# AsherBond/0-kno-blobstreamx

Hardware: AMD Instinct MI355X
Metric: Goldilocks NTT GB/s @ 2^20–2^24 (higher is better)
Workload: dtype u64; 1 GPU; forward NTT, n=2^20, batch=128 per GPU, in place, natural order (BASELINE configs[1] wires shape); log_n=20, batch_per_gpu=128, plan=strip(R=2^10,C=2^4,E=32)+finalT(R=2^10,C=2^3,E=32), plan_is_the_bit_exact_tested_plan=True

## Files before the change

### 0-kno-blobstreamx_amd/csrc/gl_field.cuh

```cuda
#pragma once
#include <stdint.h>

#if defined(__HIPCC__)
#define GL_HD __host__ __device__ __forceinline__
#else
#define GL_HD inline __attribute__((always_inline))
#endif

typedef uint64_t u64;
typedef uint32_t u32;

#define GL_P 0xFFFFFFFF00000001ULL
#define GL_EPS 0xFFFFFFFFULL

template <int V> struct glp_ic { static constexpr int value = V; };
template <int I, int N, class F>
GL_HD void glp_static_for(F&& f) {
    if constexpr (I < N) {
        f(glp_ic<I>{});
        glp_static_for<I + 1, N>(f);
    }
}

#if defined(__HIP_DEVICE_COMPILE__) && !defined(GLP_EMU) && !defined(GLP_NO_ASM_FIELD)
#define GLP_ASM_FIELD 1
#else
#define GLP_ASM_FIELD 0
#endif

GL_HD u64 gl_make64(u32 lo, u32 hi) { return ((u64)hi << 32) | lo; }

GL_HD u64 gl_add_u32(u64 x, u32 y) {
#if GLP_ASM_FIELD
    u64 r, junk;
    asm("v_mad_u64_u32 %0, %1, %2, 1, %3" : "=v"(r), "=s"(junk) : "v"(y), "v"(x));
    return r;
#else
    return x + (u64)y;
#endif
}

GL_HD u64 gl_add(u64 a, u64 b) {
    const u64 s = a + b;
    const bool over = (s < a) | (s >= GL_P);
    return s + (over ? GL_EPS : 0ULL);
}

GL_HD u64 gl_sub(u64 a, u64 b) {
#if GLP_ASM_FIELD
    u32 dl, dh;
    u64 K;
    asm("v_sub_co_u32 %0, vcc, %3, %5\n\t"
        "v_subb_co_u32 %1, vcc, %4, %6, vcc\n\t"
        "v_addc_co_u32 %0, %2, 0, %0, vcc\n\t"
        "s_andn2_b64 vcc, vcc, %2\n\t"
        "v_subbrev_co_u32 %1, %2, 0, %1, vcc"
        : "=&v"(dl), "=&v"(dh), "=&s"(K)
        : "v"((u32)a), "v"((u32)(a >> 32)), "v"((u32)b), "v"((u32)(b >> 32))
        : "scc", "vcc");
    return gl_make64(dl, dh);
#else
    u64 d = a - b;
    return (a < b) ? d - GL_EPS : d;
#endif
}

template <bool CANON>
GL_HD u64 gl_mad_eps(u32 w, u64 t) {
#if GLP_ASM_FIELD
    u64 r;
    u32 m;
    if constexpr (CANON) {
        u64 G, J;
        asm("v_mad_u64_u32 %0, vcc, %4, -1, %5\n\t"
            "v_cmp_le_u64 %1, %6, %0\n\t"
            "s_or_b64 vcc, vcc, %1\n\t"
            "s_nop 0\n\t"
            "v_cndmask_b32 %2, 0, -1, vcc\n\t"
            "v_mad_u64_u32 %0, %3, %2, 1, %0"
            : "=&v"(r), "=&s"(G), "=&v"(m), "=&s"(J)
            : "v"(w), "v"(t), "s"(GL_P)
            : "scc", "vcc");
    } else {
        u64 J;
        asm("v_mad_u64_u32 %0, vcc, %3, -1, %4\n\t"
            "v_cndmask_b32 %1, 0, -1, vcc\n\t"
            "v_mad_u64_u32 %0, %2, %1, 1, %0"
            : "=&v"(r), "=&v"(m), "=&s"(J)
            : "v"(w), "v"(t)
            : "vcc");
    }
    return r;
#else
    const u64 t1 = ((u64)w << 32) - w;
    u64 r;
    const bool c = __builtin_add_overflow(t, t1, &r);
    if (CANON) return r + ((c | (r >= GL_P)) ? GL_EPS : 0ULL);
    return r + (c ? GL_EPS : 0ULL);
#endif
}
GL_HD u64 gl_neg(u64 a) { return a ? GL_P - a : 0; }
GL_HD u64 gl_canon(u64 a) { return a >= GL_P ? a - GL_P : a; }

GL_HD u64 gl_fold_carry(u64 r, bool carry) { return r + ((carry | (r >= GL_P)) ? GL_EPS : 0ULL); }

template <bool CANON>
GL_HD u64 gl_reduce128_t(u64 hi, u64 lo) {
    const u32 h0 = (u32)hi, h1 = (u32)(hi >> 32);
#if GLP_ASM_FIELD
    u32 tl, th;
    u64 K;
    asm("v_sub_co_u32 %0, vcc, %3, %5\n\t"
        "v_subbrev_co_u32 %1, vcc, 0, %4, vcc\n\t"
        "v_addc_co_u32 %0, %2, 0, %0, vcc\n\t"
        "s_andn2_b64 vcc, vcc, %2\n\t"
        "v_subbrev_co_u32 %1, %2, 0, %1, vcc"
        : "=&v"(tl), "=&v"(th), "=&s"(K)
        : "v"((u32)lo), "v"((u32)(lo >> 32)), "v"(h1)
        : "scc", "vcc");
    return gl_mad_eps<CANON>(h0, gl_make64(tl, th));
#else
    u64 t0;
    const bool bor = __builtin_sub_overflow(lo, (u64)h1, &t0);
    t0 = bor ? t0 + GL_P : t0;
    return gl_mad_eps<CANON>(h0, t0);
#endif
}
GL_HD u64 gl_reduce128(u64 hi, u64 lo) { return gl_reduce128_t<true>(hi, lo); }

template <bool CANON>
GL_HD u64 gl_mul_t(u64 a, u64 b) {
#if !defined(__HIP_DEVICE_COMPILE__) && !defined(GLP_EMU) && defined(__SIZEOF_INT128__)
    const unsigned __int128 p = (unsigned __int128)a * b;
    return gl_reduce128_t<CANON>((u64)(p >> 64), (u64)p);
#else
    const u32 a0 = (u32)a, a1 = (u32)(a >> 32), b0 = (u32)b, b1 = (u32)(b >> 32);
    const u64 p0 = (u64)a0 * b0;
    const u64 p1 = (u64)a0 * b1 + (p0 >> 32);
    const u64 p2 = (u64)a1 * b0 + (u32)p1;
    const u64 p3 = gl_add_u32((u64)a1 * b1 + (p1 >> 32), (u32)(p2 >> 32));
    return gl_reduce128_t<CANON>(p3, (p2 << 32) | (u32)p0);
#endif
}
GL_HD u64 gl_mul(u64 a, u64 b) { return gl_mul_t<true>(a, b); }
GL_HD u64 gl_sqr(u64 a) { return gl_mul(a, a); }

GL_HD u64 gl_fold_small(u64 al, u64 ah) {
#if GLP_ASM_FIELD
    u32 lh, m;
    u64 C1, J, v;
    asm("v_add_co_u32 %0, %1, %2, %3" : "=v"(lh), "=s"(C1) : "v"((u32)(al >> 32)), "v"((u32)ah));
    asm("v_mad_u64_u32 %0, vcc, %3, -1, %4\n\t"
        "s_or_b64 vcc, vcc, %5\n\t"
        "s_nop 0\n\t"
        "v_cndmask_b32 %1, 0, -1, vcc\n\t"
        "v_mad_u64_u32 %0, %2, %1, 1, %0"
        : "=&v"(v), "=&v"(m), "=&s"(J)
        : "v"((u32)(ah >> 32)), "v"(gl_make64((u32)al, lh)), "s"(C1)
        : "scc", "vcc");
    return v;
#else
    const u64 l = al + (ah << 32);
    const bool c1 = l < al;
    const u64 t = (ah >> 32) * GL_EPS;
    const u64 v = l + t;
    const bool c2 = v < l;
    return v + ((c1 | c2) ? GL_EPS : 0ULL);
#endif
}

GL_HD u64 gl_mul_nc(u64 a, u64 b) { return gl_mul_t<false>(a, b); }

template <int T>
GL_HD u64 gl_shl_small(u64 x) {
    static_assert(T > 0 && T < 32, "");
    return gl_mad_eps<true>((u32)(x >> (64 - T)), x << T);
}
template <int K>
GL_HD u64 gl_shr_small(u64 x) {
    static_assert(K > 0 && K <= 32, "");
    const u32 m = (K == 32) ? (0u - (u32)x) : ((0u - (u32)x) & ((1u << (K & 31)) - 1u));
    const u64 a = (x + m) >> (K & 63);
    const u32 mm = (K == 32) ? m : (m << ((32 - K) & 31));
    return a + (((u64)mm << 32) - mm);
}
GL_HD u64 gl_shl32(u64 x) { return gl_mad_eps<true>((u32)(x >> 32), x << 32); }

constexpr bool gl_pow2_neg(int S) {
    const int e = S % 96;
    const bool flip = (e > 32);
    return ((S / 96) & 1) != (flip ? 1 : 0);
}
template <int S>
GL_HD u64 gl_mul_pow2_mag(u64 x) {
    static_assert(S >= 0 && S < 192, "shift out of range");
    constexpr int e = S % 96;
    if constexpr (e == 0) return x;
    else if constexpr (e < 32) return gl_shl_small<e>(x);
    else if constexpr (e == 32) return gl_shl32(x);
    else if constexpr (e < 64) return gl_shr_small<32>(gl_shr_small<64 - e>(x));
    else return gl_shr_small<96 - e>(x);
}
template <int S>
GL_HD u64 gl_mul_pow2(u64 x) {
    const u64 v = gl_mul_pow2_mag<S>(x);
    if constexpr (gl_pow2_neg(S)) return gl_neg(v);
    else return v;
}

GL_HD u64 gl_pow(u64 a, u64 e) {
    u64 r = 1;
    while (e) {
        if (e & 1) r = gl_mul(r, a);
        a = gl_mul(a, a);
        e >>= 1;
    }
    return r;
}
GL_HD u64 gl_inv(u64 a) { return gl_pow(a, GL_P - 2); }
#ifndef GLP_TWO_ADIC_GENERATOR
#define GLP_TWO_ADIC_GENERATOR 1753635133440165772ULL
#endif
#ifndef GLP_W64_LOG2
#define GLP_W64_LOG2 39
#endif
static_assert(GLP_W64_LOG2 > 0 && GLP_W64_LOG2 < 192 && GLP_W64_LOG2 % 3 == 0 && GLP_W64_LOG2 % 2 == 1, "w_64 = 2^e needs e an odd multiple of 3");
GL_HD u64 gl_root_of_unity(unsigned k) { return gl_pow(GLP_TWO_ADIC_GENERATOR, 1ULL << (32 - k)); }

struct gl_ext2 { u64 a, b; };
GL_HD gl_ext2 gl_ext_add(gl_ext2 x, gl_ext2 y) { return {gl_add(x.a, y.a), gl_add(x.b, y.b)}; }
GL_HD gl_ext2 gl_ext_sub(gl_ext2 x, gl_ext2 y) { return {gl_sub(x.a, y.a), gl_sub(x.b, y.b)}; }
GL_HD gl_ext2 gl_ext_mul(gl_ext2 x, gl_ext2 y) {
    u64 bb = gl_mul(x.b, y.b);
    u64 w = gl_add(gl_add(gl_add(bb, bb), gl_add(bb, bb)), gl_add(gl_add(bb, bb), bb));
    return {gl_add(gl_mul(x.a, y.a), w), gl_add(gl_mul(x.a, y.b), gl_mul(x.b, y.a))};
}
GL_HD gl_ext2 gl_ext_scale(gl_ext2 x, u64 s) { return {gl_mul(x.a, s), gl_mul(x.b, s)}; }
```

### 0-kno-blobstreamx_amd/csrc/ntt_kernels.cuh

```cuda
#pragma once
#include "gl_field.cuh"
#include "ntt_plan.h"

constexpr int glp_bitrev_c(int v, int bits) {
    int r = 0;
    for (int i = 0; i < bits; i++) r |= ((v >> i) & 1) << (bits - 1 - i);
    return r;
}
constexpr int glp_tw_exp(int m, int i, bool inv) {
    int e = (GLP_W64_LOG2 * (64 / m) * i) % 192;
    return inv ? (192 - e) % 192 : e;
}

template <int Q, bool INV, int OFF, int NX>
GL_HD void glp_dft_inreg(u64 (&x)[NX]) {
    glp_static_for<0, Q>([&](auto s_) {
        constexpr int s = decltype(s_)::value;
        constexpr int half = 1 << (Q - 1 - s);
        constexpr int m = 2 * half;
        glp_static_for<0, (1 << Q) / 2>([&](auto t_) {
            constexpr int t = decltype(t_)::value;
            constexpr int blk = t / half, i = t % half;
            constexpr int i0 = OFF + blk * m + i, i1 = i0 + half;
            constexpr int e = glp_tw_exp(m, i, INV);
            u64 u = x[i0], v = x[i1];
            x[i0] = gl_add(u, v);
            if constexpr (gl_pow2_neg(e)) x[i1] = gl_mul_pow2_mag<e>(gl_sub(v, u));
            else x[i1] = gl_mul_pow2_mag<e>(gl_sub(u, v));
        });
    });
}


struct GlpNttPassArgs {
    const u64* src;
    u64* dst;
    u64 src_poly_stride;
    u64 dst_poly_stride;
    const u64* tw_tile;
    const u64* tw_lo;
    const u64* tw_hi;
    u64 scale;
    u32 log_n;
    u32 log_m;
    u32 log_c;
    u32 batch;
    u32 rev;
    u32 nprev;
    u32 log_rprev[3];
    u32 xcd_group_log;
    const u64* tw_full;
    u32 poly_minor;
    u32 coset_log;
    u32 src_coset;
    const u64* in_row;
    const u64* in_col;
};

static inline bool glp_ntt_args_plain(const GlpNttPassArgs& a) {
    return !a.coset_log && !a.src_coset && !a.in_row && !a.in_col && !a.tw_full && !a.poly_minor && !a.rev;
}

template <int LOG_R, int LOG_E>
struct GlpSteps {
    static constexpr int S = (LOG_R + LOG_E - 1) / LOG_E;
    static constexpr int q(int t) { return t == 0 ? LOG_R - LOG_E * (S - 1) : LOG_E; }
    static constexpr int log_sigma(int t) { return LOG_E * (S - 1 - t); }
    static constexpr int low_bits(int t) { return t == 0 ? 0 : q(0) + LOG_E * (t - 1); }
};

template <int LOG_R, int LOG_E>
GL_HD u32 glp_digit_reverse(u32 pos) {
    using ST = GlpSteps<LOG_R, LOG_E>;
    u32 k = 0;
    glp_static_for<0, ST::S>([&](auto t_) {
        constexpr int t = decltype(t_)::value;
        u32 digit = (pos >> ST::log_sigma(t)) & ((1u << ST::q(t)) - 1u);
        k |= digit << ST::low_bits(t);
    });
    return k;
}

GL_HD u32 glp_bitrev32(u32 v, u32 bits) {
    if (bits == 0) return 0;
#if defined(__HIP_DEVICE_COMPILE__)
    return __brev(v) >> (32 - bits);
#else
    u32 r = 0;
    for (u32 i = 0; i < bits; i++) r |= ((v >> i) & 1u) << (bits - 1 - i);
    return r;
#endif
}

#if defined(GLP_EMU)
#define GLP_DYN_LDS(name) u64* name = reinterpret_cast<u64*>(glp_emu_dyn_lds())
#else
#define GLP_DYN_LDS(name) extern __shared__ __attribute__((aligned(16))) u64 name[]
#endif

template <int LOG_E, int MODE> struct GlpSplit { static constexpr bool value = (LOG_E >= 5 && MODE != GLP_FINAL_ROWS); };

template <int LOG_E, int MODE, int CT_LOG_C = -1> struct GlpBounds {
    static constexpr int threads = LOG_E == 6 ? 512 : ((LOG_E == 5 && MODE == GLP_FINAL_T) ? 256 : 1024);
    static constexpr int waves = LOG_E == 6 ? 2 : (LOG_E == 5 ? (MODE == GLP_FINAL_T ? 3 : 4) : 1);
};
template <int LOG_R, int MODE, bool INV, int LOG_E = 4, bool PLAIN = false, int CT_LOG_C = -1>
__global__ void __launch_bounds__((GlpBounds<LOG_E, MODE, CT_LOG_C>::threads), (GlpBounds<LOG_E, MODE, CT_LOG_C>::waves)) glp_ntt_pass_kernel(GlpNttPassArgs a) {
    static_assert(!PLAIN || MODE != GLP_FINAL_ROWS, "FINAL_ROWS has no plain form");
    using ST = GlpSteps<LOG_R, LOG_E>;
    const u32 a_coset_log = PLAIN ? 0u : a.coset_log;
    const u32 a_src_coset = PLAIN ? 0u : a.src_coset;
    const u64* const a_in_row = PLAIN ? nullptr : a.in_row;
    const u64* const a_in_col = PLAIN ? nullptr : a.in_col;
    const u64* const a_tw_full = PLAIN ? nullptr : a.tw_full;
    const u32 a_poly_minor = PLAIN ? 0u : a.poly_minor;
    const u32 a_rev = PLAIN ? 0u : a.rev;
    constexpr u32 R = 1u << LOG_R;
    constexpr u32 E = 1u << LOG_E;
    constexpr bool SPLIT = GlpSplit<LOG_E, MODE>::value;
    GLP_DYN_LDS(lds);
    u32* const lds32 = reinterpret_cast<u32*>(lds);

    const u32 log_c = CT_LOG_C >= 0 ? (u32)CT_LOG_C : a.log_c;
    const u32 C = 1u << log_c;
    const u32 NT = (R << log_c) >> LOG_E;
    const u32 tid = threadIdx.x;
    const u32 ldA = C + 1;
    u64 tile = blockIdx.x;
    if constexpr (MODE == GLP_STRIP || MODE == GLP_FINAL_T) {
        const u32 g = a.xcd_group_log;
        if (g) {
            const u64 per = 8ull << g;
            const u64 base = tile & ~(per - 1);
            const u32 rem = (u32)(tile & (per - 1));
            tile = base + ((u64)(rem & 7u) << g) + (rem >> 3);
        }
    }

    auto poly_off = [&](u64 v, u64 stride, bool blocked) -> u64 {
        if (!a_coset_log) return v * stride;
        const u32 kc = (u32)v & ((1u << a_coset_log) - 1u);
        return (v >> a_coset_log) * stride + (blocked ? ((u64)glp_bitrev32(kc, a_coset_log) << a.log_n) : 0ull);
    };
    const u32 coset_mask = (1u << a_coset_log) - 1u;

    u64 sbase = 0, dbase = 0;
    u32 lo0 = 0, kcos = 0;
    u64 row_first = 0;
    const u32 log_rows = a.log_n - LOG_R;
    if constexpr (MODE == GLP_STRIP) {
        const u32 log_tpp = a.log_n - LOG_R - log_c;
        u64 poly;
        u32 t;
        if (a_poly_minor) {
            const u32 g = a.xcd_group_log;
            const u64 rest = tile >> g;
            poly = rest % a.batch;
            t = (u32)(((rest / a.batch) << g) | (tile & ((1ull << g) - 1)));
        } else {
            poly = tile >> log_tpp;
            t = (u32)(tile & ((1ull << log_tpp) - 1));
        }
        const u32 log_mc = a.log_m - log_c;
        const u32 hi = t >> log_mc;
        lo0 = (t & ((1u << log_mc) - 1u)) << log_c;
        const u64 off = ((u64)hi << (LOG_R + a.log_m)) + lo0;
        sbase = poly_off(poly, a.src_poly_stride, a_src_coset != 0) + off;
        dbase = poly_off(poly, a.dst_poly_stride, true) + off;
        kcos = (u32)poly & coset_mask;
    } else {
        row_first = tile << log_c;
    }
    const u64 total_rows = (u64)a.batch << log_rows;

    u64 x[E];

    auto unit_geom = [&](auto T_, u32 g, u32& col, u32& row0, u32& o_lo) {
        constexpr int T = decltype(T_)::value;
        constexpr int q = ST::q(T);
        constexpr int lsg = ST::log_sigma(T);
        const u32 u = g * NT + tid;
        u32 o;
        if (T == 0 && MODE != GLP_STRIP) {
            o = u & ((R >> q) - 1u);
            col = u >> (LOG_R - q);
        } else {
            col = u & (C - 1u);
            o = u >> log_c;
        }
        o_lo = o & ((1u << lsg) - 1u);
        row0 = ((o >> lsg) << (q + lsg)) | o_lo;
    };

    glp_static_for<0, ST::S>([&](auto t_) {
        constexpr int t = decltype(t_)::value;
        constexpr int q = ST::q(t);
        constexpr u32 r = 1u << q;
        constexpr int lsg = ST::log_sigma(t);
        constexpr u32 G = E / r;
        constexpr bool first = (t == 0), last = (t == ST::S - 1);

        u32 colv[G], row0v[G], olov[G];
        glp_static_for<0, (int)G>([&](auto g_) {
            constexpr int g = decltype(g_)::value;
            u32 col, row0, o_lo;
            unit_geom(t_, (u32)g, col, row0, o_lo);
            colv[g] = col; row0v[g] = row0; olov[g] = o_lo;
            if constexpr (first) {
                if constexpr (MODE == GLP_STRIP) {
                    const u64* const ps = a.src + (sbase + col + ((u64)row0 << a.log_m));
                    const u64 st = 1ull << (lsg + a.log_m);
                    glp_static_for<0, (int)r>([&](auto d_) {
                        constexpr int d = decltype(d_)::value;
                        x[g * r + d] = ps[(u64)d * st];
                    });
                    if (a_in_row) {
                        u64 sc[r];
                        glp_static_for<0, (int)r>([&](auto d_) {
                            constexpr int d = decltype(d_)::value;
                            sc[d] = a_in_row[(kcos << LOG_R) + row0 + ((u32)d << lsg)];
                        });
                        glp_static_for<0, (int)r>([&](auto d_) {
                            constexpr int d = decltype(d_)::value;
                            x[g * r + d] = gl_mul(x[g * r + d], sc[d]);
                        });
                    }
                } else {
                    u64 grow = row_first + col;
                    bool active = grow < total_rows;
                    u64 poly = grow >> log_rows;
                    u32 rr = (u32)(grow & ((1ull << log_rows) - 1));
                    if constexpr (MODE == GLP_FINAL_T) {
                        u32 rem = rr, sh = log_rows, rho = 0;
                        for (u32 i = 0; i < a.nprev; i++) {
                            u32 lr = a.log_rprev[i];
                            sh -= lr;
                            rho |= (rem & ((1u << lr) - 1u)) << sh;
                            rem >>= lr;
                        }
                        rr = rho;
                    }
                    const u64 p = poly_off(poly, a.src_poly_stride, a_src_coset != 0) + ((u64)rr << LOG_R) + row0;
                    const u32 kc = (u32)poly & coset_mask;
                    glp_static_for<0, (int)r>([&](auto d_) {
                        constexpr int d = decltype(d_)::value;
                        x[g * r + d] = active ? a.src[p + ((u32)d << lsg)] : 0ull;
                    });
                    if (a_in_row) {
                        u64 sc[r];
                        glp_static_for<0, (int)r>([&](auto d_) {
                            constexpr int d = decltype(d_)::value;
                            sc[d] = a_in_row[(kc << LOG_R) + row0 + ((u32)d << lsg)];
                        });
                        glp_static_for<0, (int)r>([&](auto d_) {
                            constexpr int d = decltype(d_)::value;
                            x[g * r + d] = gl_mul(x[g * r + d], sc[d]);
                        });
                    }
                }
            } else if constexpr (!SPLIT) {
                const u32 base = row0 * ldA + col;
                glp_static_for<0, (int)r>([&](auto d_) {
                    constexpr int d = decltype(d_)::value;
                    x[g * r + d] = lds[base + ((u32)d << lsg) * ldA];
                });
            }
        });

        if constexpr (last && MODE == GLP_FINAL_ROWS && !first) __syncthreads();

        glp_static_for<0, (int)G>([&](auto g_) {
            constexpr int g = decltype(g_)::value;
            glp_dft_inreg<q, INV, g * (int)r>(x);
        });

        glp_static_for<0, (int)G>([&](auto g_) {
            constexpr int g = decltype(g_)::value;
            const u32 col = colv[g], row0 = row0v[g];
            if constexpr (!last && SPLIT) {
                const u32 o_lo = olov[g];
                u64 v[r];
                glp_static_for<0, (int)r>([&](auto d_) {
                    constexpr int d = decltype(d_)::value;
                    v[d] = x[g * r + glp_bitrev_c(d, q)];
                    if constexpr (d != 0) v[d] = gl_mul(v[d], a.tw_tile[(o_lo * (u32)d) << ST::low_bits(t)]);
                });
                glp_static_for<0, (int)r>([&](auto d_) { x[g * r + decltype(d_)::value] = v[decltype(d_)::value]; });
            } else if constexpr (!last) {
                const u32 o_lo = olov[g];
                const u32 base = row0 * ldA + col;
                glp_static_for<0, (int)r>([&](auto d_) {
                    constexpr int d = decltype(d_)::value;
                    u64 v = x[g * r + glp_bitrev_c(d, q)];
                    if constexpr (d != 0) v = gl_mul(v, a.tw_tile[(o_lo * (u32)d) << ST::low_bits(t)]);
                    lds[base + ((u32)d << lsg) * ldA] = v;
                });
            } else {
                const u32 k0 = glp_digit_reverse<LOG_R, LOG_E>(row0);
                constexpr int KS = LOG_R - q;
                if constexpr (MODE == GLP_STRIP) {
                    u64 tw = 1, ratio = 1;
                    const u64* const twf = a_tw_full;
                    if (!twf) {
                        const u32 log_N = LOG_R + a.log_m;
                        const u64 jq = (u64)(lo0 + col);
                        const u64 e0 = jq * k0;
                        const u64 e1 = jq << KS;
                        if (log_N <= 12) {
                            tw = a.tw_lo[e0];
                            ratio = a.tw_lo[e1];
                        } else {
                            tw = gl_mul(a.tw_lo[e0 & 4095u], a.tw_hi[e0 >> 12]);
                            ratio = gl_mul(a.tw_lo[e1 & 4095u], a.tw_hi[e1 >> 12]);
                        }
                        if (a_in_col) tw = gl_mul(tw, a_in_col[((u64)kcos << a.log_m) + lo0 + col]);
                    }
                    const u32 orow0 = a_rev ? glp_bitrev32(k0, LOG_R) : k0;
                    const u64 p0 = dbase + ((u64)orow0 << a.log_m) + col;
                    const u32 sh = a_rev ? a.log_m : a.log_m + KS;
                    glp_static_for<0, (int)r>([&](auto d_) {
                        constexpr int d = decltype(d_)::value;
                        u64 v = x[g * r + glp_bitrev_c(d, q)];
                        if (twf) {
                            v = gl_mul(v, twf[((u64)(k0 + ((u32)d << KS)) << a.log_m) + lo0 + col]);
                        } else {
                            v = gl_mul(v, tw);
                            if constexpr (d + 1 < (int)r) tw = gl_mul(tw, ratio);
                        }
                        const u64 dm = a_rev ? (u64)glp_bitrev_c(d, q) : (u64)d;
                        a.dst[p0 + (dm << sh)] = v;
                    });
                } else if constexpr (MODE == GLP_FINAL_T) {
                    const u64 grow = row_first + col;
                    if (grow < total_rows) {
                        const u64 poly = grow >> log_rows;
                        const u64 kappa = grow & ((1ull << log_rows) - 1);
                        const u64 p0 = poly_off(poly, a.dst_poly_stride, true) + ((u64)k0 << log_rows) + kappa;
                        const u32 sh = KS + log_rows;
                        glp_static_for<0, (int)r>([&](auto d_) {
                            constexpr int d = decltype(d_)::value;
                            u64 v = x[g * r + glp_bitrev_c(d, q)];
                            if (a.scale != 1) v = gl_mul(v, a.scale);
                            a.dst[p0 + ((u64)d << sh)] = v;
                        });
                    }
                } else {
                    const u32 kb = col * (R + 1u) + (a_rev ? glp_bitrev32(k0, LOG_R) : k0);
                    const u32 sh = a_rev ? 0u : (u32)KS;
                    glp_static_for<0, (int)r>([&](auto d_) {
                        constexpr int d = decltype(d_)::value;
                        u64 v = x[g * r + glp_bitrev_c(d, q)];
                        if (a.scale != 1) v = gl_mul(v, a.scale);
                        const u32 dm = a_rev ? (u32)glp_bitrev_c(d, q) : (u32)d;
                        lds[kb + (dm << sh)] = v;
                    });
                }
            }
        });
        if constexpr (!last && SPLIT) {
            constexpr int q2 = ST::q(t + 1);
            constexpr u32 r2 = 1u << q2;
            constexpr int lsg2 = ST::log_sigma(t + 1);
            constexpr u32 G2 = E / r2;
            u32 nb[G2];
            glp_static_for<0, (int)G2>([&](auto g_) {
                constexpr int g = decltype(g_)::value;
                u32 col, row0, o_lo;
                unit_geom(glp_ic<t + 1>{}, (u32)g, col, row0, o_lo);
                nb[g] = row0 * ldA + col;
            });
            u32 lo[E];
            glp_static_for<0, (int)G>([&](auto g_) {
                constexpr int g = decltype(g_)::value;
                const u32 base = row0v[g] * ldA + colv[g];
                glp_static_for<0, (int)r>([&](auto d_) {
                    constexpr int d = decltype(d_)::value;
                    lds32[base + ((u32)d << lsg) * ldA] = (u32)x[g * r + d];
                });
            });
            __syncthreads();
            glp_static_for<0, (int)G2>([&](auto g_) {
                constexpr int g = decltype(g_)::value;
                glp_static_for<0, (int)r2>([&](auto d_) {
                    constexpr int d = decltype(d_)::value;
                    lo[g * r2 + d] = lds32[nb[g] + ((u32)d << lsg2) * ldA];
                });
            });
            __syncthreads();
            glp_static_for<0, (int)G>([&](auto g_) {
                constexpr int g = decltype(g_)::value;
                const u32 base = row0v[g] * ldA + colv[g];
                glp_static_for<0, (int)r>([&](auto d_) {
                    constexpr int d = decltype(d_)::value;
                    lds32[base + ((u32)d << lsg) * ldA] = (u32)(x[g * r + d] >> 32);
                });
            });
            __syncthreads();
            glp_static_for<0, (int)G2>([&](auto g_) {
                constexpr int g = decltype(g_)::value;
                glp_static_for<0, (int)r2>([&](auto d_) {
                    constexpr int d = decltype(d_)::value;
                    x[g * r2 + d] = gl_make64(lo[g * r2 + d], lds32[nb[g] + ((u32)d << lsg2) * ldA]);
                });
            });
        } else if constexpr (!last || MODE == GLP_FINAL_ROWS) __syncthreads();
    });

    if constexpr (MODE == GLP_FINAL_ROWS) {
        #pragma unroll 4
        for (u32 i = tid; i < (R << log_c); i += NT) {
            const u32 col = i >> LOG_R, kk = i & (R - 1u);
            const u64 grow = row_first + col;
            if (grow < total_rows) {
                const u64 poly = grow >> log_rows;
                const u64 rr = grow & ((1ull << log_rows) - 1);
                a.dst[poly_off(poly, a.dst_poly_stride, true) + (rr << LOG_R) + kk] = lds[col * (R + 1u) + kk];
            }
        }
    }
}

template <int UNUSED = 0>
__global__ void __launch_bounds__(256) glp_ntt_small_kernel(const u64* src, u64* dst, u64 src_poly_stride,
                                                            u64 dst_poly_stride, u32 log_n, u32 batch,
                                                            const u64* tw, u64 scale, u32 rev) {
    const u32 b = blockIdx.x * blockDim.x + threadIdx.x;
    if (b >= batch) return;
    const u32 n = 1u << log_n;
    u64 in[32];
    for (u32 j = 0; j < n; j++) in[j] = src[(u64)b * src_poly_stride + j];
    for (u32 k = 0; k < n; k++) {
        u64 acc = 0;
        for (u32 j = 0; j < n; j++) acc = gl_add(acc, gl_mul(in[j], tw[(j * k) & (n - 1u)]));
        if (scale != 1) acc = gl_mul(acc, scale);
        const u32 ko = rev ? glp_bitrev32(k, log_n) : k;
        dst[(u64)b * dst_poly_stride + ko] = acc;
    }
}

template <int UNUSED = 0>
__global__ void __launch_bounds__(256) glp_build_full_tw_kernel(u64* __restrict__ full, u32 log_N, u32 log_m, const u64* __restrict__ tw_lo,
                                                                const u64* __restrict__ tw_hi) {
    const u64 N = 1ull << log_N;
    for (u64 i = (u64)blockIdx.x * blockDim.x + threadIdx.x; i < N; i += (u64)gridDim.x * blockDim.x) {
        const u64 k = i >> log_m, j = i & ((1ull << log_m) - 1);
        const u64 e = k * j;
        u64 w = tw_lo[e & 4095u];
        if (log_N > 12) w = gl_mul(w, tw_hi[e >> 12]);
        full[i] = w;
    }
}
```

### profiles/ab_ntt.py

```python
#!/usr/bin/env python3
import json
import os
import subprocess
import sys

ROOT = os.path.dirname(os.path.dirname(os.path.abspath(__file__)))
libs = sys.argv[1:]
rounds = int(os.environ.get("AB_ROUNDS", "3"))
extra = os.environ.get("AB_ARGS", "--full --no-cpu --no-sizes --no-prove --steps 30 --warmup 5").split()
for r in range(rounds):
    for lib in libs:
        env = dict(os.environ, GLP_LIB=os.path.abspath(lib))
        out = subprocess.run([sys.executable, os.path.join(ROOT, "bench.py")] + extra, env=env, stdout=subprocess.PIPE, stderr=subprocess.DEVNULL,
                             text=True).stdout.strip().splitlines()
        try:
            d = json.loads(out[-1])
            print(json.dumps({"round": r, "lib": os.path.basename(lib), "value": d["value"], "pass_ms": d["roofline"]["pass_ms_profiling_mode"],
                              "kernel_gbps": d["roofline"]["achieved"]}), flush=True)
        except Exception as e:
            print(json.dumps({"round": r, "lib": os.path.basename(lib), "error": str(e), "tail": out[-1:] }), flush=True)
```

Measured before the change: 2053 GB/s.

## Add compile-time lazy reduction plan to in-register DFT butterflies

Introduces a constexpr plan that tracks, per butterfly stage, which values must be canonical and which may stay non-canonical in [0, 2^64). Where allowed, it uses a cheaper non-canonicalizing add (gl_add_nc) and a non-canonical pow2 shift, with explicit canon fixups only where later operations need them. Twiddle generation products also switch to gl_mul_nc. This removes compare/select reduction instructions from the ALU-heavy radix kernels, at the cost of a complex invariant whose correctness relies on static_asserts and emulator instrumentation.

```diff
diff --git a/0-kno-blobstreamx_amd/csrc/gl_field.cuh b/0-kno-blobstreamx_amd/csrc/gl_field.cuh
--- a/0-kno-blobstreamx_amd/csrc/gl_field.cuh
+++ b/0-kno-blobstreamx_amd/csrc/gl_field.cuh
@@ -44,6 +44,26 @@
     const u64 s = a + b;
     const bool over = (s < a) | (s >= GL_P);
     return s + (over ? GL_EPS : 0ULL);
+}
+
+GL_HD u64 gl_add_nc(u64 a, u64 b) {
+#if GLP_ASM_FIELD
+    u32 sl, sh;
+    u64 K;
+    asm("v_add_co_u32 %0, vcc, %3, %5\n\t"
+        "v_addc_co_u32 %1, vcc, %4, %6, vcc\n\t"
+        "v_subbrev_co_u32 %0, %2, 0, %0, vcc\n\t"
+        "s_andn2_b64 vcc, vcc, %2\n\t"
+        "v_addc_co_u32 %1, %2, 0, %1, vcc"
+        : "=&v"(sl), "=&v"(sh), "=&s"(K)
+        : "v"((u32)a), "v"((u32)(a >> 32)), "v"((u32)b), "v"((u32)(b >> 32))
+        : "scc", "vcc");
+    return gl_make64(sl, sh);
+#else
+    u64 s;
+    const bool c = __builtin_add_overflow(a, b, &s);
+    return s + (c ? GL_EPS : 0ULL);
+#endif
 }
 
 GL_HD u64 gl_sub(u64 a, u64 b) {
@@ -171,35 +191,38 @@
 
 GL_HD u64 gl_mul_nc(u64 a, u64 b) { return gl_mul_t<false>(a, b); }
 
-template <int T>
+template <int T, bool CANON = true>
 GL_HD u64 gl_shl_small(u64 x) {
     static_assert(T > 0 && T < 32, "");
-    return gl_mad_eps<true>((u32)(x >> (64 - T)), x << T);
-}
-template <int K>
+    return gl_mad_eps<CANON>((u32)(x >> (64 - T)), x << T);
+}
+template <int K, bool X_CANON = true>
 GL_HD u64 gl_shr_small(u64 x) {
     static_assert(K > 0 && K <= 32, "");
+    static_assert(X_CANON, "gl_shr_small needs a canonical argument (x + m must not wrap)");
     const u32 m = (K == 32) ? (0u - (u32)x) : ((0u - (u32)x) & ((1u << (K & 31)) - 1u));
     const u64 a = (x + m) >> (K & 63);
     const u32 mm = (K == 32) ? m : (m << ((32 - K) & 31));
     return a + (((u64)mm << 32) - mm);
 }
-GL_HD u64 gl_shl32(u64 x) { return gl_mad_eps<true>((u32)(x >> 32), x << 32); }
+template <bool CANON>
+GL_HD u64 gl_shl32_t(u64 x) { return gl_mad_eps<CANON>((u32)(x >> 32), x << 32); }
+GL_HD u64 gl_shl32(u64 x) { return gl_shl32_t<true>(x); }
 
 constexpr bool gl_pow2_neg(int S) {
     const int e = S % 96;
     const bool flip = (e > 32);
     return ((S / 96) & 1) != (flip ? 1 : 0);
 }
-template <int S>
+template <int S, bool CANON = true, bool X_CANON = true>
 GL_HD u64 gl_mul_pow2_mag(u64 x) {
     static_assert(S >= 0 && S < 192, "shift out of range");
     constexpr int e = S % 96;
     if constexpr (e == 0) return x;
-    else if constexpr (e < 32) return gl_shl_small<e>(x);
-    else if constexpr (e == 32) return gl_shl32(x);
-    else if constexpr (e < 64) return gl_shr_small<32>(gl_shr_small<64 - e>(x));
-    else return gl_shr_small<96 - e>(x);
+    else if constexpr (e < 32) return gl_shl_small<e, CANON>(x);
+    else if constexpr (e == 32) return gl_shl32_t<CANON>(x);
+    else if constexpr (e < 64) return gl_shr_small<32, true>(gl_shr_small<64 - e, X_CANON>(x));
+    else return gl_shr_small<96 - e, X_CANON>(x);
 }
 template <int S>
 GL_HD u64 gl_mul_pow2(u64 x) {
diff --git a/0-kno-blobstreamx_amd/csrc/ntt_kernels.cuh b/0-kno-blobstreamx_amd/csrc/ntt_kernels.cuh
--- a/0-kno-blobstreamx_amd/csrc/ntt_kernels.cuh
+++ b/0-kno-blobstreamx_amd/csrc/ntt_kernels.cuh
@@ -12,8 +12,98 @@
     return inv ? (192 - e) % 192 : e;
 }
 
-template <int Q, bool INV, int OFF, int NX>
+#if defined(GLP_EMU)
+enum { GLP_LAZY_ADD = 0, GLP_LAZY_SUB = 1, GLP_LAZY_SHIFT = 2, GLP_LAZY_MUL = 3, GLP_LAZY_KINDS = 4 };
+inline unsigned long long glp_lazy_seen[2 * GLP_LAZY_KINDS];
+inline void glp_lazy_site(int kind, u64 v) {
+    __atomic_fetch_add(&glp_lazy_seen[2 * kind], 1ull, __ATOMIC_RELAXED);
+    if (v >= GL_P) __atomic_fetch_add(&glp_lazy_seen[2 * kind + 1], 1ull, __ATOMIC_RELAXED);
+}
+extern "C" __attribute__((used, visibility("default"))) inline void glp_emu_lazy_counts(unsigned long long* out, int reset) {
+    for (int k = 0; k < 2 * GLP_LAZY_KINDS; k++) {
+        out[k] = __atomic_load_n(&glp_lazy_seen[k], __ATOMIC_RELAXED);
+        if (reset) __atomic_store_n(&glp_lazy_seen[k], 0ull, __ATOMIC_RELAXED);
+    }
+}
+#define GLP_LAZY_SITE(kind, flagged_nc, v) do { if (flagged_nc) glp_lazy_site(kind, v); } while (0)
+#else
+#define GLP_LAZY_SITE(kind, flagged_nc, v) ((void)0)
+#endif
+
+struct GlpBfly {
+    bool fix_u, fix_v;
+    bool add_lazy;
+    bool add_fix;
+    bool swap;
+    bool tw_lazy;
+    bool tw_fix;
+    bool cu, cv;
+    bool c0, c1;
+};
+constexpr GlpBfly glp_bfly_plan(bool cu, bool cv, int e, bool n0, bool n1) {
+    GlpBfly b{};
+    const int f = e % 96;
+    const bool inverse_shift = f > 32;
+    b.swap = gl_pow2_neg(e);
+    b.fix_u = !cu && (b.swap || inverse_shift);
+    b.fix_v = !cv && (!b.swap || inverse_shift);
+    b.cu = cu || b.fix_u;
+    b.cv = cv || b.fix_v;
+    if (b.cu && b.cv && !n0) b.c0 = true;
+    else { b.add_lazy = true; b.add_fix = !n0; b.c0 = !n0; }
+    const bool cm = b.swap ? b.cv : b.cu;
+    if (inverse_shift) b.c1 = true;
+    else if (f == 0) { b.tw_fix = !cm && !n1; b.c1 = cm || b.tw_fix; }
+    else { b.tw_lazy = n1; b.c1 = !n1; }
+    return b;
+}
+constexpr int glp_bfly_lazy_operand(int e, bool n0, bool n1) {
+    const int f = e % 96;
+    if (f > 32 || !n0 || (f == 0 && !n1)) return 0;
+    return gl_pow2_neg(e) ? 2 : 1;
+}
+
+constexpr u64 glp_dft_all(int Q) { return Q >= 6 ? ~0ull : ((1ull << (1 << Q)) - 1ull); }
+template <int Q> struct GlpLazyPlan {
+    u64 may_nc[Q + 1];
+    u64 canon[Q + 1];
+};
+template <int Q, bool INV>
+constexpr GlpLazyPlan<Q> glp_lazy_plan(u64 in_canon, u64 out_may_nc) {
+    GlpLazyPlan<Q> P{};
+    P.may_nc[Q] = out_may_nc & glp_dft_all(Q);
+    for (int s = Q - 1; s >= 0; s--) {
+        const int half = 1 << (Q - 1 - s), m = 2 * half;
+        u64 allow = 0;
+        for (int t = 0; t < (1 << Q) / 2; t++) {
+            const int j0 = (t / half) * m + t % half, j1 = j0 + half;
+            const int w = glp_bfly_lazy_operand(glp_tw_exp(m, t % half, INV), (P.may_nc[s + 1] >> j0) & 1, (P.may_nc[s + 1] >> j1) & 1);
+            if (w == 1) allow |= 1ull << j0;
+            if (w == 2) allow |= 1ull << j1;
+        }
+        P.may_nc[s] = allow;
+    }
+    P.canon[0] = in_canon & glp_dft_all(Q);
+    for (int s = 0; s < Q; s++) {
+        const int half = 1 << (Q - 1 - s), m = 2 * half;
+        u64 c = 0;
+        for (int t = 0; t < (1 << Q) / 2; t++) {
+            const int j0 = (t / half) * m + t % half, j1 = j0 + half;
+            const GlpBfly b = glp_bfly_plan((P.canon[s] >> j0) & 1, (P.canon[s] >> j1) & 1, glp_tw_exp(m, t % half, INV),
+                                            (P.may_nc[s + 1] >> j0) & 1, (P.may_nc[s + 1] >> j1) & 1);
+            c |= (u64)b.c0 << j0 | (u64)b.c1 << j1;
+        }
+        P.canon[s + 1] = c;
+    }
+    return P;
+}
+template <int Q, bool INV>
+constexpr u64 glp_dft_out_canon(u64 in_canon, u64 out_may_nc) { return glp_lazy_plan<Q, INV>(in_canon, out_may_nc).canon[Q]; }
+
+template <int Q, bool INV, int OFF, u64 IN_CANON = ~0ull, u64 OUT_MAY_NC = 0ull, int NX>
 GL_HD void glp_dft_inreg(u64 (&x)[NX]) {
+    constexpr GlpLazyPlan<Q> P = glp_lazy_plan<Q, INV>(IN_CANON, OUT_MAY_NC);
+    static_assert((P.canon[Q] | P.may_nc[Q]) == glp_dft_all(Q), "an output the caller needs canonical is not");
     glp_static_for<0, Q>([&](auto s_) {
         constexpr int s = decltype(s_)::value;
         constexpr int half = 1 << (Q - 1 - s);
@@ -21,12 +111,33 @@
         glp_static_for<0, (1 << Q) / 2>([&](auto t_) {
             constexpr int t = decltype(t_)::value;
             constexpr int blk = t / half, i = t % half;
-            constexpr int i0 = OFF + blk * m + i, i1 = i0 + half;
+            constexpr int j0 = blk * m + i, j1 = j0 + half;
+            constexpr int i0 = OFF + j0, i1 = OFF + j1;
             constexpr int e = glp_tw_exp(m, i, INV);
+            constexpr GlpBfly B = glp_bfly_plan((P.canon[s] >> j0) & 1, (P.canon[s] >> j1) & 1, e, (P.may_nc[s + 1] >> j0) & 1,
+                                                (P.may_nc[s + 1] >> j1) & 1);
             u64 u = x[i0], v = x[i1];
-            x[i0] = gl_add(u, v);
-            if constexpr (gl_pow2_neg(e)) x[i1] = gl_mul_pow2_mag<e>(gl_sub(v, u));
-            else x[i1] = gl_mul_pow2_mag<e>(gl_sub(u, v));
+            if constexpr (B.fix_u) u = gl_canon(u);
+            if constexpr (B.fix_v) v = gl_canon(v);
+            if constexpr (B.add_lazy) {
+                static_assert(B.cu || B.cv, "gl_add_nc needs one canonical operand");
+                GLP_LAZY_SITE(GLP_LAZY_ADD, !B.cu, u);
+                GLP_LAZY_SITE(GLP_LAZY_ADD, !B.cv, v);
+                const u64 sum = gl_add_nc(u, v);
+                if constexpr (B.add_fix) x[i0] = gl_canon(sum);
+                else x[i0] = sum;
+            } else {
+                static_assert(B.cu && B.cv, "a canonical sum needs canonical operands");
+                x[i0] = gl_add(u, v);
+            }
+            static_assert(B.swap ? B.cu : B.cv, "gl_sub needs a canonical subtrahend");
+            constexpr bool CD = B.swap ? B.cv : B.cu;
+            GLP_LAZY_SITE(GLP_LAZY_SUB, !CD, B.swap ? v : u);
+            const u64 d = B.swap ? gl_sub(v, u) : gl_sub(u, v);
+            GLP_LAZY_SITE(GLP_LAZY_SHIFT, !CD && e % 96 != 0, d);
+            const u64 w = gl_mul_pow2_mag<e, !B.tw_lazy, CD>(d);
+            if constexpr (B.tw_fix) x[i1] = gl_canon(w);
+            else x[i1] = w;
         });
     });
 }
@@ -199,6 +310,10 @@
         constexpr int lsg = ST::log_sigma(t);
         constexpr u32 G = E / r;
         constexpr bool first = (t == 0), last = (t == ST::S - 1);
+        constexpr u64 ALL = glp_dft_all(q);
+        constexpr u64 OUT_MAY_NC = last ? (MODE == GLP_STRIP ? ALL : 0ull) : (ALL & ~1ull);
+        constexpr u64 OUT_CANON = glp_dft_out_canon<q, INV>(ALL, OUT_MAY_NC);
+        static_assert(last ? (MODE == GLP_STRIP || OUT_CANON == ALL) : (OUT_CANON & 1ull), "a value stored without a product must be canonical");
 
         u32 colv[G], row0v[G], olov[G];
         glp_static_for<0, (int)G>([&](auto g_) {
@@ -271,7 +386,7 @@
 
         glp_static_for<0, (int)G>([&](auto g_) {
             constexpr int g = decltype(g_)::value;
-            glp_dft_inreg<q, INV, g * (int)r>(x);
+            glp_dft_inreg<q, INV, g * (int)r, ALL, OUT_MAY_NC>(x);
         });
 
         glp_static_for<0, (int)G>([&](auto g_) {
@@ -283,6 +398,7 @@
                 glp_static_for<0, (int)r>([&](auto d_) {
                     constexpr int d = decltype(d_)::value;
                     v[d] = x[g * r + glp_bitrev_c(d, q)];
+                    GLP_LAZY_SITE(GLP_LAZY_MUL, d != 0 && !((OUT_CANON >> glp_bitrev_c(d, q)) & 1), v[d]);
                     if constexpr (d != 0) v[d] = gl_mul(v[d], a.tw_tile[(o_lo * (u32)d) << ST::low_bits(t)]);
                 });
                 glp_static_for<0, (int)r>([&](auto d_) { x[g * r + decltype(d_)::value] = v[decltype(d_)::value]; });
@@ -292,6 +408,7 @@
                 glp_static_for<0, (int)r>([&](auto d_) {
                     constexpr int d = decltype(d_)::value;
                     u64 v = x[g * r + glp_bitrev_c(d, q)];
+                    GLP_LAZY_SITE(GLP_LAZY_MUL, d != 0 && !((OUT_CANON >> glp_bitrev_c(d, q)) & 1), v);
                     if constexpr (d != 0) v = gl_mul(v, a.tw_tile[(o_lo * (u32)d) << ST::low_bits(t)]);
                     lds[base + ((u32)d << lsg) * ldA] = v;
                 });
@@ -310,10 +427,10 @@
                             tw = a.tw_lo[e0];
                             ratio = a.tw_lo[e1];
                         } else {
-                            tw = gl_mul(a.tw_lo[e0 & 4095u], a.tw_hi[e0 >> 12]);
-                            ratio = gl_mul(a.tw_lo[e1 & 4095u], a.tw_hi[e1 >> 12]);
+                            tw = gl_mul_nc(a.tw_lo[e0 & 4095u], a.tw_hi[e0 >> 12]);
+                            ratio = gl_mul_nc(a.tw_lo[e1 & 4095u], a.tw_hi[e1 >> 12]);
                         }
-                        if (a_in_col) tw = gl_mul(tw, a_in_col[((u64)kcos << a.log_m) + lo0 + col]);
+                        if (a_in_col) tw = gl_mul_nc(tw, a_in_col[((u64)kcos << a.log_m) + lo0 + col]);
                     }
                     const u32 orow0 = a_rev ? glp_bitrev32(k0, LOG_R) : k0;
                     const u64 p0 = dbase + ((u64)orow0 << a.log_m) + col;
@@ -321,11 +438,12 @@
                     glp_static_for<0, (int)r>([&](auto d_) {
                         constexpr int d = decltype(d_)::value;
                         u64 v = x[g * r + glp_bitrev_c(d, q)];
+                        GLP_LAZY_SITE(GLP_LAZY_MUL, !((OUT_CANON >> glp_bitrev_c(d, q)) & 1), v);
                         if (twf) {
                             v = gl_mul(v, twf[((u64)(k0 + ((u32)d << KS)) << a.log_m) + lo0 + col]);
                         } else {
                             v = gl_mul(v, tw);
-                            if constexpr (d + 1 < (int)r) tw = gl_mul(tw, ratio);
+                            if constexpr (d + 1 < (int)r) tw = gl_mul_nc(tw, ratio);
                         }
                         const u64 dm = a_rev ? (u64)glp_bitrev_c(d, q) : (u64)d;
                         a.dst[p0 + (dm << sh)] = v;
diff --git a/profiles/ab_ntt.py b/profiles/ab_ntt.py
--- a/profiles/ab_ntt.py
+++ b/profiles/ab_ntt.py
@@ -11,8 +11,12 @@
 for r in range(rounds):
     for lib in libs:
         env = dict(os.environ, GLP_LIB=os.path.abspath(lib))
-        out = subprocess.run([sys.executable, os.path.join(ROOT, "bench.py")] + extra, env=env, stdout=subprocess.PIPE, stderr=subprocess.DEVNULL,
-                             text=True).stdout.strip().splitlines()
+        run = subprocess.run([sys.executable, os.path.join(ROOT, "bench.py")] + extra, env=env, stdout=subprocess.PIPE, stderr=subprocess.DEVNULL,
+                             text=True, timeout=int(os.environ.get("AB_TIMEOUT", "180")))
+        out = run.stdout.strip().splitlines()
+        if run.returncode != 0:
+            print(json.dumps({"round": r, "lib": os.path.basename(lib), "error": f"bench.py exited {run.returncode}", "tail": out[-1:]}), flush=True)
+            sys.exit(1)
         try:
             d = json.loads(out[-1])
             print(json.dumps({"round": r, "lib": os.path.basename(lib), "value": d["value"], "pass_ms": d["roofline"]["pass_ms_profiling_mode"],
```

New measurement: 2059 GB/s (median of 6 runs). Within noise of the previous version (+0.2%).
